# nlapier2/Metalign

Measured on AMD Instinct MI355X. Metric: 150bp reads/s end-to-end (CMash filter + profile), higher is better.
Workload: dtype u64; 1 GPU; configs[2]: 10M reads vs 10k-genome DB, multi-k {21,31,51} containment — 10000000 synthetic 150bp reads/GPU vs 10000-genome sketch DB (50000 bp genomes, n=1000), k in [21, 31, 51], 12498882 alignment records/GPU, 10001 taxa, 1 MI355X per rank; inputs resident in HBM; stage_a_definition=reference_pipeline, hash_mode=0, stage_a_match=kmer

## Files before the change

### metalign_amd/csrc/mg_kcount_core.h

```cpp
#pragma once
#include <cstdint>
#include <utility>

#ifdef MG_HOST_CHECK
#define MG_LDS
#define MG_GLB
#define MG_HD static inline
#define MG_UNIFORM(x) (x)
#else
#include <hip/hip_runtime.h>
#define MG_LDS __attribute__((address_space(3)))
#define MG_GLB __attribute__((address_space(1)))
#define MG_HD __device__ __forceinline__
#define MG_UNIFORM(x) ((uint32_t)__builtin_amdgcn_readfirstlane((int)(x)))
#endif

#ifdef MG_HOST_CHECK
#define MG_KC_ADD(ptr, v) ((*(ptr) += (v)) - (v))
#define MG_KC_OR(ptr, v) (*(ptr) |= (v))
#define MG_KC_AND(ptr, v) (*(ptr) &= (v))
#define MG_KC_LOAD(ptr) (*(ptr))
#define MG_KC_CAS(ptr, expected, desired) (*(ptr) = (*(ptr) == (expected)) ? (desired) : *(ptr))
#else
#ifdef MG_KC_PLAIN_LOADS
#define MG_KC_LOAD(ptr) (*(ptr))
#else
#define MG_KC_LOAD(ptr) __hip_atomic_load((ptr), __ATOMIC_RELAXED, __HIP_MEMORY_SCOPE_AGENT)
#endif
#define MG_KC_ADD(ptr, v) __hip_atomic_fetch_add((ptr), (v), __ATOMIC_RELAXED, __HIP_MEMORY_SCOPE_AGENT)
#define MG_KC_OR(ptr, v) __hip_atomic_fetch_or((ptr), (v), __ATOMIC_RELAXED, __HIP_MEMORY_SCOPE_AGENT)
#define MG_KC_AND(ptr, v) __hip_atomic_fetch_and((ptr), (v), __ATOMIC_RELAXED, __HIP_MEMORY_SCOPE_AGENT)
#define MG_KC_CAS(ptr, expected, desired)                                                                                          \
  do {                                                                                                                             \
    uint32_t mg_kc_expected_ = (expected);                                                                                         \
    (void)__hip_atomic_compare_exchange_strong((ptr), &mg_kc_expected_, (desired), __ATOMIC_RELAXED, __ATOMIC_RELAXED,             \
                                               __HIP_MEMORY_SCOPE_AGENT);                                                          \
  } while (0)
#endif

namespace mg {

constexpr int kKcM = 15;
constexpr uint32_t kKcMask = 0x3fffffffu;
constexpr uint32_t kKcNone = 0xffffffffu;
constexpr uint32_t kKcXor = 0x1b873593u & kKcMask;
constexpr uint32_t kKcMul = 0x2545f491u;
constexpr uint32_t kKcPos = 1023u;
constexpr int kKcMinK = kKcM, kKcMaxK = 64;
constexpr int kKcMaxCands = 50;
constexpr uint32_t kKcSeveral = 0xffu;
constexpr uint32_t kKcSlots = 4;
constexpr uint32_t kKcMaxRead = 1023;

constexpr int kc_flank(int k) { return k >= 53 ? 2 + (k - 51) / 2 : (k >= 23 ? 2 : (k >= 19 ? 1 : 0)); }
constexpr int kc_cands(int k) { return k - kKcM + 1 - 2 * kc_flank(k); }

MG_HD uint32_t kc_word(uint32_t f, uint32_t r, uint32_t pos) {
  const uint32_t c = f < r ? f : r;
  return (((c ^ kKcXor) >> 8) << 10) | pos;
}
MG_HD uint32_t kc_rc32(uint32_t x);
MG_HD uint32_t kc_ext_hash(uint64_t v, int k) {
  const int nb = 2 * (kKcM + 2 * kc_flank(k));
  const uint64_t f = v >> (64 - nb);
  const uint64_t r = ((((uint64_t)kc_rc32((uint32_t)v)) << 32) | kc_rc32((uint32_t)(v >> 32))) & ((1ull << nb) - 1ull);
  const uint64_t c = f < r ? f : r;
  const uint32_t hi = (uint32_t)(c >> 32);
#ifdef MG_HOST_CHECK
  uint32_t h = (uint32_t)c * 0x9E3779B1u + (hi & 0xffffffu) * 0x85EBCBu + (hi >> 24) * 0xC2B2AFu;
#else
  uint32_t h = (uint32_t)c * 0x9E3779B1u + __umul24(hi & 0xffffffu, 0x85EBCBu) + __umul24(hi >> 24, 0xC2B2AFu);
#endif
  h ^= h >> 15; h *= 0x2C1B3C6Du;
  h ^= h >> 13;
  return h & 0xfffffffeu;
}
constexpr uint32_t kKcGateExtra = 5;
constexpr uint32_t kc_gate_bits(uint64_t nd, uint32_t extra) {
  uint32_t b = 0;
  while (b < 32u && (1ull << b) < nd) ++b;
  b += extra;
  return b < 16u ? 16u : (b > 32u ? 32u : b);
}


MG_HD uint32_t kc_ext32(const MG_LDS uint32_t* s, uint32_t p) {
  const uint32_t d = p >> 4, sh = (p & 15u) << 1;
  const uint64_t v = ((uint64_t)s[d] << 32) | s[d + 1];
  return (uint32_t)((v << sh) >> 32);
}
MG_HD uint32_t kc_bits32(const MG_LDS uint32_t* s, uint32_t p) {
  const uint32_t d = p >> 5, sh = p & 31u;
  const uint64_t v = ((uint64_t)s[d] << 32) | s[d + 1];
  return (uint32_t)((v << sh) >> 32);
}

MG_HD uint64_t kc_ext64(const MG_LDS uint32_t* s, uint32_t p) {
  const uint32_t d = p >> 4, sh = (p & 15u) << 1;
  const uint32_t a = s[d], b = s[d + 1], c = s[d + 2];
#ifdef MG_HOST_CHECK
  const uint32_t hi = (uint32_t)(((((uint64_t)a) << 32 | b) << sh) >> 32), lo = (uint32_t)(((((uint64_t)b) << 32 | c) << sh) >> 32);
#else
  const uint32_t n = (sh ^ 31u) + 1u;
  const uint32_t hi = sh ? __builtin_amdgcn_alignbit(a, b, n) : a, lo = sh ? __builtin_amdgcn_alignbit(b, c, n) : b;
#endif
  return ((uint64_t)hi << 32) | lo;
}
MG_HD uint32_t kc_run_hash(const MG_LDS uint32_t* fwd, uint32_t p0, uint32_t pos, int k) {
  return kc_ext_hash(kc_ext64(fwd, p0 + pos), k);
}
MG_HD uint32_t kc_event(uint32_t word, uint32_t info) { return (word << 20) | info; }
MG_HD uint32_t kc_event_first(uint32_t ev, uint32_t& next) {
  const uint32_t out = (ev & ~1023u) | next;
  next = ((ev >> 10) & 1023u) + 1u;
  return out;
}
MG_HD bool kc_event_none(uint32_t ev) { return ((ev >> 20) & kKcPos) == kKcPos; }
MG_HD uint32_t kc_event_pos(uint32_t ev) { return (ev >> 20) & kKcPos; }

struct KcWin { uint32_t w[4]; };

MG_HD uint32_t kc_keep_mask(int k, int word) {
  const int nb = 2 * k - 32 * word;
  return nb <= 0 ? 0u : (nb >= 32 ? 0xffffffffu : 0xffffffffu << (32 - nb));
}

MG_HD KcWin kc_ext128(const MG_LDS uint32_t* s, uint32_t p, int k) {
  const uint32_t d = p >> 4, sh = (p & 15u) << 1;
  uint32_t a[5];
#pragma unroll
  for (int i = 0; i < 5; ++i) a[i] = s[d + i];
  KcWin x;
#pragma unroll
  for (int i = 0; i < 4; ++i) x.w[i] = (uint32_t)(((((uint64_t)a[i]) << 32 | a[i + 1]) << sh) >> 32) & kc_keep_mask(k, i);
  return x;
}

MG_HD bool kc_less(const KcWin& a, const KcWin& b) {
#pragma unroll
  for (int i = 0; i < 3; ++i)
    if (a.w[i] != b.w[i]) return a.w[i] < b.w[i];
  return a.w[3] < b.w[3];
}
MG_HD bool kc_equal(const KcWin& a, const KcWin& b) {
  return a.w[0] == b.w[0] && a.w[1] == b.w[1] && a.w[2] == b.w[2] && a.w[3] == b.w[3];
}

MG_HD uint32_t kc_rev2(uint32_t x) {
#ifdef MG_HOST_CHECK
  x = ((x >> 1) & 0x55555555u) | ((x & 0x55555555u) << 1);
  x = ((x >> 2) & 0x33333333u) | ((x & 0x33333333u) << 2);
  x = ((x >> 4) & 0x0f0f0f0fu) | ((x & 0x0f0f0f0fu) << 4);
  x = ((x >> 8) & 0x00ff00ffu) | ((x & 0x00ff00ffu) << 8);
  x = (x >> 16) | (x << 16);
#else
  x = __builtin_bitreverse32(x);
#endif
  return ((x >> 1) & 0x55555555u) | ((x & 0x55555555u) << 1);
}
MG_HD uint32_t kc_rc32(uint32_t x) { return kc_rev2(~x); }

MG_HD KcWin kc_revcomp(const KcWin& x, int k) {
  const uint32_t r[4] = {kc_rc32(x.w[3]), kc_rc32(x.w[2]), kc_rc32(x.w[1]), kc_rc32(x.w[0])};
  const int s = 2 * (64 - k);
  KcWin o;
#pragma unroll
  for (int i = 0; i < 4; ++i) {
    const int q = i + (s >> 5), sh = s & 31;
    const uint32_t hi = q < 4 ? r[q < 4 ? q : 3] : 0u, lo = q + 1 < 4 ? r[q + 1 < 4 ? q + 1 : 3] : 0u;
    o.w[i] = (sh ? (hi << sh) | (lo >> (32 - sh)) : hi) & kc_keep_mask(k, i);
  }
  return o;
}

MG_HD KcWin kc_from_right(uint64_t hi, uint64_t lo, int k) {
  const int s = 128 - 2 * k;
  uint64_t h, l;
  if (s == 0) { h = hi; l = lo; }
  else if (s < 64) { h = (hi << s) | (lo >> (64 - s)); l = lo << s; }
  else { h = s == 64 ? lo : lo << (s - 64); l = 0; }
  return KcWin{{(uint32_t)(h >> 32), (uint32_t)h, (uint32_t)(l >> 32), (uint32_t)l}};
}

MG_HD KcWin kc_canonical(const KcWin& x, int k) {
  const KcWin r = kc_revcomp(x, k);
  return kc_less(r, x) ? r : x;
}

MG_HD uint32_t kc_mmer_at(const KcWin& x, int j) {
  const int d = j >> 4, sh = (j & 15) << 1;
  const uint64_t v = ((uint64_t)x.w[d] << 32) | (d + 1 < 4 ? x.w[d + 1 < 4 ? d + 1 : 3] : 0u);
  return (uint32_t)((v << sh) >> 34);
}
MG_HD uint32_t kc_mmer_rc(uint32_t f) { return kc_rc32(f << 2) & kKcMask; }

MG_HD uint64_t kc_sub64(const KcWin& x, int j) {
  const int d = j >> 4, sh = (j & 15) << 1;
  const uint32_t a = x.w[d < 4 ? d : 3], b = d + 1 < 4 ? x.w[d + 1 < 4 ? d + 1 : 3] : 0u, c = d + 2 < 4 ? x.w[d + 2 < 4 ? d + 2 : 3] : 0u;
  const uint32_t hi = (uint32_t)(((((uint64_t)a) << 32 | b) << sh) >> 32), lo = (uint32_t)(((((uint64_t)b) << 32 | c) << sh) >> 32);
  return ((uint64_t)hi << 32) | lo;
}

MG_HD int kc_table_keys(const KcWin& x, int k, uint32_t* out) {
  const int e = kc_flank(k), w = kc_cands(k);
  uint32_t best = kKcNone;
  for (int j = 0; j < w; ++j) {
    const uint32_t f = kc_mmer_at(x, j + e);
    const uint32_t rank = kc_word(f, kc_mmer_rc(f), 0u);
    best = rank < best ? rank : best;
  }
  int n = 0;
  for (int j = 0; j < w; ++j) {
    const uint32_t f = kc_mmer_at(x, j + e);
    if (kc_word(f, kc_mmer_rc(f), 0u) != best) continue;
    const uint32_t h = kc_ext_hash(kc_sub64(x, j), k);
    bool seen = false;
    for (int t = 0; t < n; ++t) seen = seen || out[t] == h;
    if (!seen) out[n++] = h;
  }
  return n;
}
MG_HD uint32_t kc_table_key_offset(const KcWin& x, int k, uint32_t h) {
  const int e = kc_flank(k), w = kc_cands(k);
  uint32_t best = kKcNone, off = kKcSeveral;
  for (int j = 0; j < w; ++j) {
    const uint32_t f = kc_mmer_at(x, j + e);
    const uint32_t rank = kc_word(f, kc_mmer_rc(f), 0u);
    best = rank < best ? rank : best;
  }
  int n = 0;
  for (int j = 0; j < w; ++j) {
    const uint32_t f = kc_mmer_at(x, j + e);
    if (kc_word(f, kc_mmer_rc(f), 0u) != best || kc_ext_hash(kc_sub64(x, j), k) != h) continue;
    off = (uint32_t)j;
    ++n;
  }
  return n == 1 ? off : kKcSeveral;
}

struct __attribute__((aligned(16))) KcEntry {
  uint32_t w[4];
  uint32_t head;
  uint32_t key;
  uint32_t off;
  uint32_t pad;
};

MG_HD uint32_t kc_pack4(uint32_t x, uint32_t& nz) {
  const uint32_t u = x & 0xDFDFDFDFu;
  const uint32_t t = (x >> 1) & 0x03030303u;
  const uint32_t c = t ^ ((t >> 1) & 0x01010101u);
#ifdef MG_HOST_CHECK
  uint32_t letters = 0;
  for (int b = 0; b < 4; ++b) letters |= ((0x54474341u >> (8 * ((c >> (8 * b)) & 3u))) & 0xffu) << (8 * b);
#else
  const uint32_t letters = __builtin_amdgcn_perm(0u, 0x54474341u, c);
#endif
  nz = letters ^ u;
  return (c * 0x40100401u) >> 24;
}
MG_HD uint32_t kc_pack16(const uint32_t v[4], uint32_t& notbase) {
  uint32_t n0, n1, n2, n3;
  const uint32_t p = (kc_pack4(v[0], n0) << 24) | (kc_pack4(v[1], n1) << 16) | (kc_pack4(v[2], n2) << 8) | kc_pack4(v[3], n3);
  notbase = n0 | n1 | n2 | n3;
  return p;
}
MG_HD uint32_t kc_notbase16(const uint32_t v[4]) {
  uint32_t out = 0;
#pragma unroll
  for (int i = 0; i < 4; ++i) {
    uint32_t nz;
    (void)kc_pack4(v[i], nz);
    const uint32_t b = ((((nz & 0x7F7F7F7Fu) + 0x7F7F7F7Fu) | nz) >> 7) & 0x01010101u;
    out = (out << 4) | (((b * 0x08040201u) >> 24) & 0xFu);
  }
  return out;
}

template <int K, int MODE, class Out>
MG_HD uint32_t kc_walk(const MG_LDS uint32_t* fwd, const MG_LDS uint32_t* inv, uint32_t p0, uint32_t len, uint32_t maxlen, uint32_t w0,
                       Out& out, uint32_t& cnt) {
  constexpr int M = kKcM, E = kc_flank(K), W = kc_cands(K);
  constexpr uint32_t kCap = Out::kCap;
  static_assert(K >= kKcMinK && K <= kKcMaxK, "k out of range for the minimizer path");
  maxlen = MG_UNIFORM(maxlen);
  w0 = MG_UNIFORM(w0);
  if (maxlen < (uint32_t)K) return 0u;
  const uint32_t nw = len >= (uint32_t)K ? len - (uint32_t)K + 1u : 0u;
  const uint32_t nwmax = maxlen - (uint32_t)K + 1u;
  if (w0 >= nwmax) return nwmax;
  const uint32_t nmers = nwmax + (uint32_t)(W - 1);
  uint32_t f = 0, r = 0, vrun = 0;
  p0 += (uint32_t)E;
  uint32_t word = kc_ext32(fwd, p0 + (w0 & ~15u)), iw = 0;
  if constexpr (MODE == 0) iw = kc_bits32(inv, p0 + (w0 & ~31u));
  uint32_t A[W];
  uint32_t P = kKcNone, Mprev = kKcNone;
  auto take = [&](uint32_t u) -> uint32_t {
    if ((u & 15u) == 0) word = kc_ext32(fwd, p0 + u);
    const uint32_t c = (word >> (30u - 2u * (u & 15u))) & 3u;
    f = (f << 2) | (c << 2);
#ifdef MG_HOST_CHECK
    r = (r >> 2) | ((c ^ 3u) << 30);
#else
    r = __builtin_amdgcn_alignbit(c ^ 3u, r, 2);
#endif
    const uint32_t ct = f < r ? f : r;
    uint32_t key = (ct & ~kKcPos) ^ (((kKcXor << 2) & ~kKcPos) | (u - (uint32_t)(M - 1)));
    if constexpr (MODE == 0) {
      if ((u & 31u) == 0) iw = kc_bits32(inv, p0 + u);
      const uint32_t bad = (iw >> (31u - (u & 31u))) & 1u;
      vrun = bad ? 0u : vrun + 1u;
      key = vrun >= (uint32_t)M ? key : kKcNone;
    }
    return key;
  };
  for (uint32_t u = w0; u + 1 < w0 + (uint32_t)M; ++u) (void)take(u);
  [&]<int... T>(std::integer_sequence<int, T...>) {
    ((A[T] = take(w0 + (uint32_t)(T + M - 1)), P = T == 0 ? A[T] : (A[T] < P ? A[T] : P)), ...);
  }(std::make_integer_sequence<int, W>{});
  Mprev = P;
  if constexpr (MODE != 1) Mprev = w0 < nw ? Mprev : kKcNone;
  uint32_t walked = w0 + 1u;
  for (uint32_t b = 1;; ++b) {
    if constexpr (W > 2) {
      [&]<int... T>(std::integer_sequence<int, T...>) {
        ((A[W - 2 - T] = A[W - 2 - T] < A[W - 1 - T] ? A[W - 2 - T] : A[W - 1 - T]), ...);
      }(std::make_integer_sequence<int, W - 2>{});
    }
    const uint32_t j0 = w0 + b * (uint32_t)W;
    if (j0 >= nmers || out.any_full(cnt)) break;
    const bool tail = j0 + (uint32_t)W > nmers;
    auto step = [&]<int T, bool ENDS>() -> bool {
      const uint32_t j = j0 + (uint32_t)T;
      if constexpr (ENDS && T % 8 == 0 && T > 0) { if (j >= nmers) return false; }
      const uint32_t key = take(j + (uint32_t)M - 1u);
      P = T == 0 ? key : (key < P ? key : P);
      uint32_t Mc = P;
      if constexpr (T != W - 1) { const uint32_t s = A[T + 1 < W ? T + 1 : 0]; Mc = s < P ? s : P; }
      const uint32_t i = j - (uint32_t)(W - 1);
      if constexpr (MODE != 1 || ENDS) Mc = i < nw ? Mc : kKcNone;
      out.put(cnt, Mprev, ((i - 1u) & 1023u) << 10);
      const bool ch = Mc != Mprev;
      cnt += ch ? 1u : 0u;
      cnt = cnt < kCap ? cnt : kCap;
      Mprev = Mc;
      A[T] = key;
      walked = i + 1u;
      return true;
    };
    bool whole;
    if (tail)
      whole = [&]<int... T>(std::integer_sequence<int, T...>) { return (step.template operator()<T, true>() && ...); }(
          std::make_integer_sequence<int, W>{});
    else
      whole = [&]<int... T>(std::integer_sequence<int, T...>) { return (step.template operator()<T, false>() && ...); }(
          std::make_integer_sequence<int, W>{});
    if (!whole) break;
  }
  walked = walked < nwmax ? walked : nwmax;
  out.put(cnt, Mprev, ((walked - 1u) & 1023u) << 10);
  cnt += cnt < kCap ? 1u : 0u;
  const uint32_t safe = cnt >= kCap ? out.last_window(kCap - 1u) + 1u : walked;
  return out.wave_min(safe < walked ? safe : walked);
}

MG_HD uint32_t kc_clean_windows(const MG_LDS uint32_t* inv, uint32_t p0, uint32_t len, uint32_t maxlen, int k) {
  uint32_t vrun = 0, n = 0, iw = 0;
  for (uint32_t u = 0; u < maxlen; ++u) {
    if ((u & 31u) == 0) iw = kc_bits32(inv, p0 + u);
    const uint32_t bad = (iw >> (31u - (u & 31u))) & 1u;
    vrun = bad ? 0u : vrun + 1u;
    n += (vrun >= (uint32_t)k && u < len) ? 1u : 0u;
  }
  return n;
}

struct KcIndexView {
  MG_GLB uint32_t* live;
  const MG_GLB uint32_t* shared;
  const MG_GLB KcEntry* prim;
  const MG_GLB KcEntry* ovf;
  MG_GLB uint32_t* counts;
  MG_GLB uint32_t* csat;
  uint32_t bmask;
  uint32_t gshift;
  uint32_t cs;
  uint32_t ablate;
  uint32_t epoch;
};

MG_HD uint32_t kc_entry_count(uint32_t word, uint32_t epoch) { return (word >> 24) == epoch ? (word & 0xffffffu) : 0u; }

#ifdef MG_HOST_CHECK
MG_HD KcEntry kc_load_entry(const KcEntry* ent, uint32_t e) { return ent[e]; }
#else
typedef uint32_t kc_u32x4 __attribute__((ext_vector_type(4)));
MG_HD KcEntry kc_load_entry(const MG_GLB KcEntry* ent, uint32_t e) {
  const MG_GLB kc_u32x4* p = reinterpret_cast<const MG_GLB kc_u32x4*>(ent + e);
  const kc_u32x4 a = p[0], b = p[1];
  return KcEntry{{a.x, a.y, a.z, a.w}, b.x, b.y, b.z, b.w};
}
#endif
MG_HD KcEntry kc_entry(const KcIndexView& ix, uint32_t n) {
  const uint32_t nprim = kKcSlots * (ix.bmask + 1u);
  return n < nprim ? kc_load_entry(ix.prim, n) : kc_load_entry(ix.ovf, n - nprim);
}

MG_HD bool kc_gate(const KcIndexView& ix, uint32_t key) {
  const uint32_t g = key >> ix.gshift;
  return (MG_KC_LOAD(&ix.live[g >> 5]) >> (g & 31u)) & 1u;
}

MG_HD bool kc_window_clean(const MG_LDS uint32_t* inv, uint32_t p, int k) {
  const uint32_t d = p >> 5, sh = p & 31u;
  const uint32_t a = inv[d], b = inv[d + 1], c = inv[d + 2];
  const uint32_t v0 = (uint32_t)(((((uint64_t)a) << 32 | b) << sh) >> 32), v1 = (uint32_t)(((((uint64_t)b) << 32 | c) << sh) >> 32);
  const uint32_t m0 = k >= 32 ? 0xffffffffu : 0xffffffffu << (32 - k);
  const uint32_t m1 = k <= 32 ? 0u : (k >= 64 ? 0xffffffffu : 0xffffffffu << (64 - k));
  return ((v0 & m0) | (v1 & m1)) == 0u;
}


MG_HD uint32_t kc_scan_run(const MG_LDS uint32_t* fwd, const MG_LDS uint32_t* inv, int k, bool bad, const uint32_t* ew,
                           uint32_t p0, uint32_t i1, uint32_t i2) {
  constexpr int NS = 5;
  const uint32_t p = p0 + i1, d = p >> 4, sh = (p & 15u) << 1;
  uint32_t w[NS];
  {
    uint32_t a[NS + 1];
#pragma unroll
    for (int j = 0; j < NS + 1; ++j) a[j] = fwd[d + j];
#pragma unroll
    for (int j = 0; j < NS; ++j) w[j] = (uint32_t)(((((uint64_t)a[j]) << 32 | a[j + 1]) << sh) >> 32);
  }
  const uint32_t sigmask = kc_keep_mask(k, 0);
  const uint32_t sig_rc = kc_revcomp(KcWin{{ew[0], ew[1], ew[2], ew[3]}}, k).w[0];
  uint64_t hits = 0;
  for (uint32_t i = i1; i <= i2; ++i) {
    const uint32_t x0 = w[0] & sigmask;
    hits |= (x0 == ew[0] || x0 == sig_rc) ? 1ull << (i - i1) : 0ull;
#pragma unroll
    for (int j = 0; j < NS - 1; ++j) w[j] = (w[j] << 2) | (w[j + 1] >> 30);
    w[NS - 1] <<= 2;
  }
  uint32_t found = 0;
  while (hits) {
    const uint32_t i = i1 + (uint32_t)__builtin_ctzll(hits);
    hits &= hits - 1;
    if (bad && !kc_window_clean(inv, p0 + i, k)) continue;
    const KcWin x = kc_ext128(fwd, p0 + i, k), y = kc_revcomp(x, k);
    const KcWin c = kc_less(y, x) ? y : x;
    found += (c.w[0] == ew[0] && c.w[1] == ew[1] && c.w[2] == ew[2] && c.w[3] == ew[3]) ? 1u : 0u;
  }
  return found;
}

MG_HD uint32_t kc_match_windows(const MG_LDS uint32_t* fwd, const MG_LDS uint32_t* inv, int k, bool bad, uint32_t e0, uint32_t e1,
                                uint32_t e2, uint32_t e3, uint32_t off, uint32_t p0, uint32_t pos, uint32_t i1, uint32_t i2) {
  const uint32_t wc = (uint32_t)kc_cands(k);
  const uint32_t ia = pos - off, ib = pos - (wc - 1u - off);
  const uint32_t sigmask = kc_keep_mask(k, 0);
  uint32_t found = 0;
  if (ia >= i1 && ia <= i2 && (kc_ext32(fwd, p0 + ia) & sigmask) == e0 && !(bad && !kc_window_clean(inv, p0 + ia, k))) {
    const KcWin x = kc_ext128(fwd, p0 + ia, k);
    found += (x.w[0] == e0 && x.w[1] == e1 && x.w[2] == e2 && x.w[3] == e3) ? 1u : 0u;
  }
  if (ib >= i1 && ib <= i2 && !(ib == ia && found) && !(bad && !kc_window_clean(inv, p0 + ib, k))) {
    const uint32_t tail = kc_rc32(kc_ext32(fwd, p0 + ib + (uint32_t)k - 16u));
    if (k < 16 || (tail & sigmask) == e0) {
      const KcWin y = kc_revcomp(kc_ext128(fwd, p0 + ib, k), k);
      found += (y.w[0] == e0 && y.w[1] == e1 && y.w[2] == e2 && y.w[3] == e3) ? 1u : 0u;
    }
  }
  return found;
}

MG_HD void kc_count_entry(const KcIndexView& ix, uint32_t n, uint32_t head, uint32_t found, uint32_t seen) {
  if (!found || ix.ablate == 5u) return;
  (void)MG_KC_ADD(&ix.counts[head], found);
  if (ix.cs) {
    if ((seen >> 24) == ix.epoch) (void)MG_KC_ADD(&ix.csat[n], found);
    else MG_KC_CAS(&ix.csat[n], seen, (ix.epoch << 24) | found);
  }
}

MG_HD uint32_t kc_match_run(const KcIndexView& ix, const MG_LDS uint32_t* fwd, const MG_LDS uint32_t* inv, int k, bool bad, uint32_t key,
                            uint32_t p0, uint32_t pos, uint32_t i1, uint32_t i2) {
  const uint32_t b = key & ix.bmask, nprim = kKcSlots * (ix.bmask + 1u);
  uint32_t found = 0, novf = 0, ovf_at = 0;
  bool any = false, open = false;
  for (uint32_t t = 0; t < kKcSlots + novf; ++t) {
    const uint32_t n = t < kKcSlots ? kKcSlots * b + t : nprim + ovf_at + (t - kKcSlots);
    const KcEntry E = kc_entry(ix, n);
    if (t == 0) novf = E.pad;
    if (t == 1) ovf_at = E.pad;
    if (E.key != key) continue;
    any = true;
    const uint32_t seen = MG_KC_LOAD(&ix.csat[n]);
    if (ix.cs && kc_entry_count(seen, ix.epoch) >= ix.cs) continue;
    open = true;
    const uint32_t f = E.off == kKcSeveral ? kc_scan_run(fwd, inv, k, bad, E.w, p0, i1, i2)
                                           : kc_match_windows(fwd, inv, k, bad, E.w[0], E.w[1], E.w[2], E.w[3], E.off, p0, pos, i1, i2);
    kc_count_entry(ix, n, E.head, f, seen);
    found += f;
  }
  const uint32_t g = key >> ix.gshift;
  if (ix.cs && any && !open && !((ix.shared[g >> 5] >> (g & 31u)) & 1u) && ((MG_KC_LOAD(&ix.live[g >> 5]) >> (g & 31u)) & 1u))
    MG_KC_AND(&ix.live[g >> 5], ~(1u << (g & 31u)));
  return found;
}

}
```

Baseline: 4.561 billion reads/s.

## Add 32-aligned block minimizer walk with prefetched packed words for k with 32/33 candidates

Adds a specialized minimizer window walk for k values whose candidate count is 32 or 33. It starts at a 32-aligned base so every per-position phase is a compile-time constant, and it prefetches the next packed LDS words a few positions ahead instead of calling the generic extract helper. It also fuses the invalid-base check to phase 0. The aim is to cut the per-nucleotide index arithmetic and LDS load latency in the hot k-mer scan. In exchange the code gets larger, and there is masked-start handling whose correctness depends on the alignment edge cases.

```diff
diff --git a/metalign_amd/csrc/mg_kcount_core.h b/metalign_amd/csrc/mg_kcount_core.h
--- a/metalign_amd/csrc/mg_kcount_core.h
+++ b/metalign_amd/csrc/mg_kcount_core.h
@@ -277,9 +277,16 @@
   return out;
 }
 
+#ifdef MG_KC_WALK33
+constexpr bool kKcAlignedBlocks = false;
+#else
+constexpr bool kKcAlignedBlocks = true;
+#endif
+constexpr bool kc_has_aligned_blocks(int k) { return kKcAlignedBlocks && (kc_cands(k) == 32 || kc_cands(k) == 33); }
+
 template <int K, int MODE, class Out>
-MG_HD uint32_t kc_walk(const MG_LDS uint32_t* fwd, const MG_LDS uint32_t* inv, uint32_t p0, uint32_t len, uint32_t maxlen, uint32_t w0,
-                       Out& out, uint32_t& cnt) {
+MG_HD uint32_t kc_walk_any(const MG_LDS uint32_t* fwd, const MG_LDS uint32_t* inv, uint32_t p0, uint32_t len, uint32_t maxlen, uint32_t w0,
+                           Out& out, uint32_t& cnt) {
   constexpr int M = kKcM, E = kc_flank(K), W = kc_cands(K);
   constexpr uint32_t kCap = Out::kCap;
   static_assert(K >= kKcMinK && K <= kKcMaxK, "k out of range for the minimizer path");
@@ -365,6 +372,109 @@
   return out.wave_min(safe < walked ? safe : walked);
 }
 
+constexpr int kKcAhead = 8;
+template <int K, int MODE, class Out>
+MG_HD uint32_t kc_walk32(const MG_LDS uint32_t* fwd, const MG_LDS uint32_t* inv, uint32_t p0, uint32_t len, uint32_t maxlen, uint32_t w0,
+                         Out& out, uint32_t& cnt) {
+  constexpr int M = kKcM, E = kc_flank(K), W = kc_cands(K), B = 32, D = W - B;
+  constexpr uint32_t kCap = Out::kCap;
+  constexpr uint32_t kXor = (kKcXor << 2) & ~kKcPos;
+  static_assert(D == 0 || D == 1, "blocks of 32 serve windows of 32 or 33 candidates");
+  maxlen = MG_UNIFORM(maxlen);
+  w0 = MG_UNIFORM(w0);
+  if (maxlen < (uint32_t)K) return 0u;
+  const uint32_t nw = len >= (uint32_t)K ? len - (uint32_t)K + 1u : 0u;
+  const uint32_t nwmax = maxlen - (uint32_t)K + 1u;
+  if (w0 >= nwmax) return nwmax;
+  const uint32_t nmers = nwmax + (uint32_t)(W - 1);
+  const uint32_t base = w0 & ~31u;
+  const bool masked = base != w0;
+  const uint32_t nwl = nw > w0 ? nw - w0 : 0u;
+  uint32_t f = 0, r = 0, vrun = 0;
+  p0 += (uint32_t)E;
+  const uint32_t d0 = p0 >> 4, sh = (p0 & 15u) << 1;
+  uint32_t word = 0, na = fwd[d0 + (base >> 4)], nb = fwd[d0 + (base >> 4) + 1u], iw = 0;
+  auto take = [&]<int PH>(uint32_t u, uint32_t kj) -> uint32_t {
+    if constexpr ((PH & 15) == 0) word = (uint32_t)(((((uint64_t)na) << 32 | nb) << sh) >> 32);
+    if constexpr ((PH & 15) == 16 - kKcAhead) { na = fwd[d0 + (u >> 4) + 1u]; nb = fwd[d0 + (u >> 4) + 2u]; }
+    const uint32_t c = (word >> (30 - 2 * (PH & 15))) & 3u;
+    f = (f << 2) | (c << 2);
+#ifdef MG_HOST_CHECK
+    r = (r >> 2) | ((c ^ 3u) << 30);
+#else
+    r = __builtin_amdgcn_alignbit(c ^ 3u, r, 2);
+#endif
+    const uint32_t ct = f < r ? f : r;
+    uint32_t key = (ct & ~kKcPos) ^ kj;
+    if constexpr (MODE == 0) {
+      if constexpr (PH == 0) iw = kc_bits32(inv, p0 + u);
+      const uint32_t bad = (iw >> (31 - PH)) & 1u;
+      vrun = bad ? 0u : vrun + 1u;
+      key = vrun >= (uint32_t)M ? key : kKcNone;
+    }
+    return key;
+  };
+  [&]<int... T>(std::integer_sequence<int, T...>) {
+    ((void)take.template operator()<T>(base + (uint32_t)T, 0u), ...);
+  }(std::make_integer_sequence<int, M - 1>{});
+  uint32_t A[B];
+  uint32_t P = kKcNone, Mprev = kKcNone;
+  if constexpr (D == 1) Mprev = take.template operator()<M - 1>(base + (uint32_t)(M - 1), kXor + base);
+  [&]<int... T>(std::integer_sequence<int, T...>) {
+    ((A[T] = take.template operator()<(D + T + M - 1) & 31>(base + (uint32_t)(D + T + M - 1), kXor + base + (uint32_t)(D + T)),
+      P = T == 0 ? A[T] : (A[T] < P ? A[T] : P)), ...);
+  }(std::make_integer_sequence<int, B>{});
+  Mprev = P < Mprev ? P : Mprev;
+  Mprev = base - w0 < nwl ? Mprev : kKcNone;
+  uint32_t walked = base + 1u;
+  for (uint32_t b = 1;; ++b) {
+    [&]<int... T>(std::integer_sequence<int, T...>) {
+      ((A[B - 2 - T] = A[B - 2 - T] < A[B - 1 - T] ? A[B - 2 - T] : A[B - 1 - T]), ...);
+    }(std::make_integer_sequence<int, B - 2 + D>{});
+    const uint32_t i0 = base + 1u + (b - 1u) * (uint32_t)B;
+    const uint32_t j0 = i0 + (uint32_t)(W - 1);
+    if (j0 >= nmers || out.any_full(cnt)) break;
+    const bool tail = j0 + (uint32_t)B > nmers;
+    const uint32_t kb = kXor + j0, ib = ((i0 - 1u) & 1023u) << 10, vb = i0 - w0;
+    auto step = [&]<int T, bool ENDS>() -> bool {
+      if constexpr (ENDS && T % 8 == 0 && T > 0) { if (j0 + (uint32_t)T >= nmers) return false; }
+      const uint32_t key = take.template operator()<(D + T + M - 1) & 31>(j0 + (uint32_t)(T + M - 1), kb + (uint32_t)T);
+      P = T == 0 ? key : (key < P ? key : P);
+      uint32_t Mc = P;
+      if constexpr (D == 1 || T != B - 1) { const uint32_t s = A[D == 1 ? T : (T + 1 < B ? T + 1 : 0)]; Mc = s < P ? s : P; }
+      if constexpr (MODE != 1 || ENDS) Mc = vb + (uint32_t)T < nwl ? Mc : kKcNone;
+      out.put(cnt, Mprev, ib + ((uint32_t)T << 10));
+      const bool ch = Mc != Mprev;
+      cnt += ch ? 1u : 0u;
+      cnt = cnt < kCap ? cnt : kCap;
+      Mprev = Mc;
+      A[T] = key;
+      walked = i0 + (uint32_t)T + 1u;
+      return true;
+    };
+    bool whole;
+    if (tail || (MODE == 1 && masked))
+      whole = [&]<int... T>(std::integer_sequence<int, T...>) { return (step.template operator()<T, true>() && ...); }(
+          std::make_integer_sequence<int, B>{});
+    else
+      whole = [&]<int... T>(std::integer_sequence<int, T...>) { return (step.template operator()<T, false>() && ...); }(
+          std::make_integer_sequence<int, B>{});
+    if (!whole) break;
+  }
+  walked = walked < nwmax ? walked : nwmax;
+  out.put(cnt, Mprev, ((walked - 1u) & 1023u) << 10);
+  cnt += cnt < kCap ? 1u : 0u;
+  const uint32_t safe = cnt >= kCap ? out.last_window(kCap - 1u) + 1u : walked;
+  return out.wave_min(safe < walked ? safe : walked);
+}
+
+template <int K, int MODE, class Out>
+MG_HD uint32_t kc_walk(const MG_LDS uint32_t* fwd, const MG_LDS uint32_t* inv, uint32_t p0, uint32_t len, uint32_t maxlen, uint32_t w0,
+                       Out& out, uint32_t& cnt) {
+  if constexpr (kc_has_aligned_blocks(K)) return kc_walk32<K, MODE>(fwd, inv, p0, len, maxlen, w0, out, cnt);
+  else return kc_walk_any<K, MODE>(fwd, inv, p0, len, maxlen, w0, out, cnt);
+}
+
 MG_HD uint32_t kc_clean_windows(const MG_LDS uint32_t* inv, uint32_t p0, uint32_t len, uint32_t maxlen, int k) {
   uint32_t vrun = 0, n = 0, iw = 0;
   for (uint32_t u = 0; u < maxlen; ++u) {
```

Result: faster. 4.712 billion reads/s, median of 6 (+3.3%).
